# facebookresearch/wmar

Hardware: AMD Instinct MI355X
Metric: watermarked images/sec at 256x256 (16x16 tok), batch 64; detector p-value delta vs ref (higher is better)
Workload: dtype f32; 1 GPU; Taming cin_transformer (48L x 1536d x 24h, V=16384) + VQGAN f16/16384, 256x256, batch 64 per GPU, greenlist watermark delta=2 gamma=0.25 h=1 (linear/stratifiedrand), T=1 top-k 250 top-p 0.92; sample -> decode -> re-encode -> detect; random-init weights; batch_per_gpu=64, decode_loop=hipGraph replay, backend=nccl

## Files before the change

### wmar_amd/csrc/gpt.hip

```cpp
#include <cstdint>
#include <map>
#include <string>
#include <vector>

#include "decoder_host.h"
#include "decode_small.h"


using namespace wmar;

struct LayerW {
    float4 *wqkv, *wproj, *wfc1, *wfc2;
    float4* wfc1x16 = nullptr;
    float2* wfc1x8 = nullptr;
    float4* wqkvx_bx = nullptr;
    float4* wproj_bx = nullptr;
    float *bqkv, *bproj, *bfc1, *bfc2, *cqkv, *cfc1;
};

struct SmallW {
    float *wqkv = nullptr, *wproj = nullptr, *wfc1 = nullptr, *wfc2 = nullptr, *ln1w = nullptr, *ln2w = nullptr;
};

struct wmar_gpt {
// ... 15 lines not shown
    double* stats_q = nullptr;
    float *kcache = nullptr, *vcache = nullptr;
    float *logits = nullptr, *scratch = nullptr;
    long long* past = nullptr;
    int *pos_dev = nullptr, *step_dev = nullptr;
    hipEvent_t ev0 = nullptr;
    static constexpr int N_PHASE = 3;
    GraphSlots<N_PHASE> gr;
    GraphSlots<N_PHASE + 1> grh;
    unsigned long long hook_key[12] = {0};
    int att_nw = 2;
    unsigned long long graph_key[12] = {0};
    int att_t1 = 1 << 30, att_t2 = 1 << 30;
    bool att_user = false;
    int att_phase(int kv, int64_t B) const {
        if (!att_user && B * H < 512) return kv <= 128 ? 1 : 2;
        return kv <= att_t1 ? 0 : (kv <= att_t2 ? 1 : 2);
    }
    static int phase_waves(int ph) { return ph == 0 ? 1 : (ph == 1 ? 2 : 4); }
    int timing = 0;
    bool no_bx_qkv = false, no_bx_proj = false;
    unsigned* xsync = nullptr;
    bool xcd_ok = false;
    bool xcd_ok_created = false;
    bool no_xr = false;
    int inject_fail = 0;
    int fallbacks = 0;
    unsigned long long* dbg_sums = nullptr; int dbg_slot = 0;
    unsigned long long* stamps = nullptr;
    unsigned long long* stamp_slot(int l, int role) const {
        return stamps ? stamps + ((long long)(l * 5 + role) * WMAR_STAMP_UNITS) * 8 : nullptr;
    }
    bool no_bx = false;
    int force_s[3] = {0, 0, 0};
    double step_ms = 0.0;
    struct Span { int cls; hipEvent_t a, b; };
    std::vector<Span> spans;
    std::vector<hipEvent_t> ev_pool;
    size_t ev_used = 0;
    bool span_on = false;
    double cls_us[WMAR_T_NCLASS] = {0};
    int64_t cls_calls[WMAR_T_NCLASS] = {0};
    hipEvent_t next_event() {
        if (ev_used == ev_pool.size()) {
            hipEvent_t e = nullptr;
            (void)hipEventCreate(&e);
            ev_pool.push_back(e);
        }
        return ev_pool[ev_used++];
    }
    void span_begin(int cls, hipStream_t st) {
        if (!span_on) return;
        Span s{cls, next_event(), next_event()};
        (void)hipEventRecord(s.a, st);
        spans.push_back(s);
    }
    void span_end(hipStream_t st) {
        if (!span_on) return;
        (void)hipEventRecord(spans.back().b, st);
    }
    void span_collect() {
        for (int i = 0; i < WMAR_T_NCLASS; ++i) { cls_us[i] = 0; cls_calls[i] = 0; }
        for (auto& s : spans) {
            float ms = 0.f;
            if (hipEventElapsedTime(&ms, s.a, s.b) == hipSuccess) { cls_us[s.cls] += ms * 1000.0; cls_calls[s.cls] += 1; }
        }
// ... 53 lines not shown
        r.slabs = g->slabs; r.slab_stride = act;
        xcur = g->x;
        S_qkv = g->force_s[0] > 0 ? (g->force_s[0] > QKV_SLABS_MAX ? QKV_SLABS_MAX : g->force_s[0]) : 1;
        S_proj = g->force_s[1] > 0 ? g->force_s[1] : split_for(D / 32, KBD);
        S_fc2 = g->force_s[2] > 0 ? g->force_s[2] : ((MT % 2 == 0 && KBF >= 128) ? 4 : split_for(D / 32, KBF));
        if (g->force_s[2] <= 0 && MT == 2 && KBF >= 256) {
            const int NTd = D / 32;
            const int Slo = 256 / NTd;
            if (Slo >= 2 && Slo < MAX_SLABS && NTd * Slo <= 256) { S_fc2 = Slo; fc2_hi = 256 - NTd * Slo; if (fc2_hi >= NTd) fc2_hi = 0; }
        }
        const int NTq = 3 * D / 32;
        if (g->force_s[0] <= 0 && NTq % 4 == 0 && MT <= 2 && S_fc2 + (fc2_hi > 0 ? 1 : 0) <= MAX_SLABS) {
            const int G = NTq / 4;
            int S = 256 / G;
            if (S > QKV_SLABS_MAX) S = QKV_SLABS_MAX;
            if (S > KBD / QX_CK) S = KBD / QX_CK;
            if (S >= 1) S_qx = S;
        }
        proj_bx = MT == 2 && g->yq && g->layers[0].wproj_bx && !g->no_bx && !g->no_bx_proj && g->force_s[1] <= 0;
        if (proj_bx) S_proj = D / BX_KSLICE;
        proj_xr = xr_shape() && g->xcd_ok;
        nch_ln2 = proj_xr ? 16 : nch;
    }
    void dbg(const void* p, long long bytes) {
#ifdef WMAR_DEV_KNOBS
        if (!g->dbg_sums || g->dbg_slot >= 4096) return;
        hipLaunchKernelGGL(k_dbg_sum, dim3(512), dim3(256), 0, st, (const uint32_t*)p, bytes / 4, g->dbg_sums + g->dbg_slot++);
#else
        (void)p; (void)bytes;
#endif
    }
    bool xr_shape() const { return proj_bx && !g->no_xr && S_proj == 4 && (D / 32) % 8 == 0 && (D / 32 / 8) * S_proj <= 32 && (D / 32 / 8) % 2 == 0; }
    bool qkv_bx() const { return S_qx > 0 && MT == 2 && g->layers[0].wqkvx_bx && !g->no_bx && !g->no_bx_qkv; }
    bool fc1_x() const { return MT == 2 && g->layers[0].wfc1x16 && nch_ln2 <= 16; }
    int qx_nkeep() const { const int G = 3 * D / 128; return G >= 4 && S_qx * 4 <= STAT_CHUNKS_MAX ? 4 : 1; }
    bool head_ntw2() const { const int NT = g->V / 32; return MT == 2 && NT % 2 == 0 && NT / 2 <= 512; }
    int head_per() const { const int MG = (MT % 2 == 0) ? MT / 2 : MT; return 256 / MG > 0 ? 256 / MG : 1; }
    int split_for(int NT, int KB) const { return pick_split(MT % 2 == 0 ? NT * (MT / 2) : NT * MT, KB, 4); }
    GemmArgs base() const {
        GemmArgs a{};
        a.MT = MT; a.B = (int)B; a.stats = g->stats; a.n_chunks = nch; a.K = D;
        return a;
    }
    SgArgs sg_base() const {
        SgArgs a{};
        a.pos_dev = g->pos_dev; a.D = D; a.H = g->H; a.Tmax = g->Tmax;
        return a;
    }
    int embed() {
        if (small) {
            SeArgs e{g->tok_emb, g->pos_emb, g->xs, io.tok, io.tok_stride, io.tok_use_pos, g->pos_dev, D};
            g->span_begin(WMAR_T_EMBED, st);
            hipLaunchKernelGGL(k_sembed, dim3((unsigned)((D / 4 + 255) / 256), (unsigned)B), dim3(256), 0, st, e);
            g->span_end(st);
            return launch_status("k_sembed");
        }
        r.x = xcur;
        g->span_begin(WMAR_T_EMBED, st);
        hipLaunchKernelGGL((k_resid_stats<true, 0>), dim3(nch * MT), dim3(256), 0, st, r);
        g->span_end(st);
        return launch_status("k_resid_stats<embed>");
    }
    int resid(const float* bias, int S, int n_hi = 0) {
        r.x = xcur;
        r.S = S + (n_hi > 0 ? 1 : 0); r.bias = bias; r.n_hi = n_hi;
        g->span_begin(WMAR_T_RESID, st);
// ... 239 lines not shown
        const long long actb = act * 16, Mpad = MT * 32;
        const long long lstride = (long long)g->Bmax * g->H * g->Tmax * g->hd;
        switch (s) {
            case WMAR_GPT_STAGE_EMBED: dbg(xcur, actb); dbg(g->stats, nch * Mpad * 16); break;
            case WMAR_GPT_STAGE_QKV:
                if (S_qx > 0) { dbg(xcur, actb); dbg(g->stats_q, S_qx * Mpad * 16); dbg(g->qkv_slabs, S_qx * 3 * actb); }
                else { dbg(xcur, actb); dbg(g->stats, nch * Mpad * 16); dbg(g->qkv_slabs, 3 * actb); }
                break;
            case WMAR_GPT_STAGE_ATTN:
                if (proj_bx) dbg(g->yq, (long long)D / 16 * 2 * 3 * 64 * 16); else dbg(g->y, actb);
                dbg(g->kcache + l * lstride, lstride * 4); dbg(g->vcache + l * lstride, lstride * 4);
                break;
            case WMAR_GPT_STAGE_PROJ:
                dbg(g->slabs, S_proj * actb);
                if (proj_xr) { dbg(xcur, actb); dbg(g->stats, nch_ln2 * Mpad * 16); }
                break;
            case WMAR_GPT_STAGE_RESID_ATTN: dbg(xcur, actb); dbg(g->stats, nch_ln2 * Mpad * 16); break;
            case WMAR_GPT_STAGE_FC1: dbg(g->hbuf, 4 * actb); break;
            case WMAR_GPT_STAGE_FC2: dbg(g->slabs, S_fc2 * actb); break;
            case WMAR_GPT_STAGE_RESID_OUT: dbg(xcur, actb); dbg(g->stats, nch * Mpad * 16); break;
            default: break;
        }
    }
    int run_stages(int first, int last, int l) {
        for (int s = first; s <= last; ++s) {
            if (!has_stage(s, l)) continue;
            if (int rc = run_stage(s, l)) return rc;
            dbg_stage(s, l);
        }
        return WMAR_OK;
    }
};

int enqueue_step(wmar_gpt* g, int64_t B, const StepIO& io, hipStream_t st) {
    StepPlan p(g, B, io, st);
    int rc;
#ifdef WMAR_DEV_KNOBS
    if (g->dbg_sums) { g->dbg_slot = 0; if (hipMemsetAsync(g->dbg_sums, 0, 4096 * 8, st) != hipSuccess) return WMAR_EHIP; }
#endif
    if ((rc = p.run_stages(WMAR_GPT_STAGE_EMBED, WMAR_GPT_STAGE_EMBED, 0))) return rc;
    for (int l = 0; l < g->L; ++l)
        if ((rc = p.run_stages(WMAR_GPT_STAGE_RESID_IN, WMAR_GPT_STAGE_FC2, l))) return rc;
    return p.run_stages(WMAR_GPT_STAGE_RESID_OUT, WMAR_GPT_STAGE_HEAD, g->L - 1);
}

void note_replayed(wmar_gpt* g, int64_t B, const StepIO& io) {
    StepPlan pl(g, B, io, nullptr);
    if (!pl.small && pl.proj_xr) g->xr_enqueued = true;
}

}

extern "C" {

int wmar_gpt_create(const wmar_gpt_config* cfg, const char* const* names, const void* const* tensors_dev,
                    int32_t n_tensors, void* stream, wmar_gpt** out) {
    WMAR_REQUIRE(cfg && names && tensors_dev && out, "gpt_create: null argument");
    WMAR_REQUIRE(cfg->n_embd % cfg->n_head == 0, "n_embd %% n_head != 0");
    const int D = cfg->n_embd, H = cfg->n_head, hd = D / H, V = cfg->vocab_size, L = cfg->n_layer;
    WMAR_REQUIRE(D % 32 == 0 && V % 32 == 0 && D <= 8192, "n_embd (<= 8192) and vocab_size must be multiples of 32 (got %d, %d)", D, V);
    WMAR_REQUIRE(hd == 32 || hd == 64 || hd == 128, "head_dim %d unsupported (32, 64, 128)", hd);
    WMAR_REQUIRE(cfg->max_batch >= 1 && cfg->max_batch <= 128, "max_batch must be in 1..128");
    WMAR_REQUIRE(cfg->block_size >= 1 && L >= 1, "bad block_size / n_layer");
    TensorMap tm(names, tensors_dev, n_tensors);
    hipStream_t st = (hipStream_t)stream;
    auto* g = new wmar_gpt();
    g->cfg = *cfg; g->D = D; g->H = H; g->hd = hd; g->V = V; g->L = L; g->Tmax = cfg->block_size; g->Bmax = cfg->max_batch;
    g->MTmax = mt_for(cfg->max_batch);
#ifdef WMAR_DEV_KNOBS
    {
        const char* names_s[3] = {"WMAR_S_QKV", "WMAR_S_PROJ", "WMAR_S_FC2"};
        for (int i = 0; i < 3; ++i) {
            const char* e = getenv(names_s[i]);
            if (e) g->force_s[i] = atoi(e) > MAX_SLABS ? MAX_SLABS : atoi(e);
        }
    }
#endif
    g->no_bx = getenv("WMAR_NO_BX") != nullptr;
#ifdef WMAR_STAMPS
    if (getenv("WMAR_STAMPS")) {
        const size_t n = (size_t)L * 5 * WMAR_STAMP_UNITS * 8;
        if (hipMalloc(&g->stamps, n * 8) != hipSuccess || hipMemset(g->stamps, 0, n * 8) != hipSuccess) g->stamps = nullptr;
    }
#endif
#ifdef WMAR_DEV_KNOBS
    if (getenv("WMAR_DBG_SUMS")) { if (hipMalloc(&g->dbg_sums, 4096 * 8) != hipSuccess) g->dbg_sums = nullptr; }
    g->no_bx_qkv = getenv("WMAR_NO_BX_QKV") != nullptr; g->no_bx_proj = getenv("WMAR_NO_BX_PROJ") != nullptr;
#endif
    int& rc = tm.rc;
    const float* te = tm.need("tok_emb.weight");
    const float* pe = tm.need("pos_emb");
    const float* hw = tm.need("head.weight");
    const float *lfw = tm.need("ln_f.weight"), *lfb = tm.need("ln_f.bias");
    if (rc == WMAR_OK) {
        WMAR_TRY(copy_vec(g, &g->tok_emb, te, (size_t)V * D, st));
        WMAR_TRY(copy_vec(g, &g->pos_emb, pe, (size_t)cfg->block_size * D, st));
        WMAR_TRY(g->mem.alloc(&g->whead, (size_t)V * D / 4));
        WMAR_TRY(pack(hw, g->whead, V, D, 0, st, lfw));
        WMAR_TRY(g->mem.alloc(&g->bhead, (size_t)V));
        WMAR_TRY(fold_bias(hw, nullptr, lfb, g->bhead, V, D, st));
        WMAR_TRY(g->mem.alloc(&g->chead, (size_t)V));
        WMAR_TRY(fold_bias(hw, nullptr, lfw, g->chead, V, D, st));
    }
    g->layers.resize(L);
    for (int l = 0; l < L && rc == WMAR_OK; ++l) {
        std::string p = "blocks." + std::to_string(l) + ".";
        LayerW& w = g->layers[l];
        const float *qw = tm.need(p + "attn.query.weight"), *kw = tm.need(p + "attn.key.weight"), *vw = tm.need(p + "attn.value.weight");
        const float *qb = tm.need(p + "attn.query.bias"), *kb = tm.need(p + "attn.key.bias"), *vb = tm.need(p + "attn.value.bias");
        const float *pw = tm.need(p + "attn.proj.weight"), *pb = tm.need(p + "attn.proj.bias");
        const float *f1w = tm.need(p + "mlp.0.weight"), *f1b = tm.need(p + "mlp.0.bias");
// ... 190 lines not shown
            case WMAR_T_RESID: if (p.small) { set_error("profile_role: the small-batch path has no residual launch"); return WMAR_EINVAL; } return p.resid(g->layers[l].bproj, p.S_proj);
            case WMAR_T_FC1: return p.fc1(l);
            case WMAR_T_FC2: return p.fc2(l);
            case WMAR_T_HEAD: return p.head();
            default: set_error("profile_role: unknown role %d", role); return WMAR_EINVAL;
        }
    };
    const bool was = g->span_on;
    g->span_on = false;
    int rc = WMAR_OK;
    for (int i = 0; i < 3 && rc == WMAR_OK; ++i) rc = one(i);
    if (rc == WMAR_OK && hipEventRecord(g->ev0, st) != hipSuccess) rc = WMAR_EHIP;
    for (int i = 0; i < iters && rc == WMAR_OK; ++i) rc = one(i + 3);
    if (rc == WMAR_OK && hipEventRecord(g->gr.done, st) != hipSuccess) rc = WMAR_EHIP;
    g->span_on = was;
    if (rc) return rc;
    WMAR_HIP_CHECK(hipEventSynchronize(g->gr.done));
    float ms = 0.f;
    WMAR_HIP_CHECK(hipEventElapsedTime(&ms, g->ev0, g->gr.done));
    *avg_us = (double)ms * 1000.0 / iters;
    return WMAR_OK;
}

int wmar_gpt_plan_info(wmar_gpt* g, int64_t B, char* buf, int64_t buf_len) {
    WMAR_REQUIRE(g && buf && buf_len > 0, "plan_info: null argument");
    WMAR_REQUIRE(B >= 1 && B <= g->Bmax, "plan_info: batch outside 1..%d", g->Bmax);
    StepIO io{g->past, (long long)g->Tmax + 1, 0, g->logits};
    StepPlan p(g, B, io, nullptr);
    if (p.small) {
        const int n = snprintf(buf, (size_t)buf_len,
                               "qkv=k_sgemv<QKV> (row-major weight stream, LN1 + bias + cache append inside, %d columns per workgroup);"
                               "attn=k_sattn (4 waves per (sequence, head));proj=k_sgemv<PROJ> (residual added in place);resid=none;"
                               "resid_launches_per_step=0;fc1=k_sgemv<FC1> (LN2 + bias + GELU inside);fc2=k_sgemv<FC2> (8 K segments, residual added in place);"
                               "head=k_sgemv<HEAD> (ln_f inside);barrier_fallbacks=%d;path=small-batch streaming (decode_small.h)",
                               sg_cols_wg<3, 3, SG_QKV>(), g->fallbacks);
        WMAR_REQUIRE(n > 0 && n < buf_len, "plan_info: buffer of %lld bytes too small", (long long)buf_len);
        return WMAR_OK;
    }
    char qkv[96], proj[160], fc1[96], fc2[96];
    const int S_in = p.S_fc2 + (p.fc2_hi > 0 ? 1 : 0);
    if (p.qkv_bx()) snprintf(qkv, sizeof qkv, "k_qkvx_bx<%d> (bf16 pipe, %d K slices)", S_in, p.S_qx);
    else if (p.S_qx > 0) snprintf(qkv, sizeof qkv, "k_qkvx<%d,%d> (fp32 MFMA, %d K slices)", p.MT, S_in, p.S_qx);
    else snprintf(qkv, sizeof qkv, "k_gemm<EPI_PACKED> (fp32 MFMA, %d K slices) after k_resid_stats", p.S_qkv);
    if (p.proj_xr) snprintf(proj, sizeof proj, "k_bx_xr<%d,4> (bf16 pipe, 4 K slices + XCD-local reduction: residual fold and LN2 statistics inside)", BX_PER);
    else if (p.proj_bx) snprintf(proj, sizeof proj, "k_bx<1,%d> (bf16 pipe, %d K slices)", BX_PER, p.S_proj);
    else snprintf(proj, sizeof proj, "k_gemm<EPI_PACKED> (fp32 MFMA, %d K slices)", p.S_proj);
    if (p.fc1_x()) snprintf(fc1, sizeof fc1, "k_fc1x (fp32 MFMA, 24-column tiles, whole K)");
    else snprintf(fc1, sizeof fc1, "k_gemm<EPI_GELU,LN> (fp32 MFMA, whole K)");
    snprintf(fc2, sizeof fc2, "k_gemm<EPI_PACKED> (fp32 MFMA, %d%s K slices)", p.S_fc2, p.fc2_hi > 0 ? "/+1" : "");
    char attn[96];
    const int w0 = wmar_gpt::phase_waves(g->att_phase(1, B)), w1 = wmar_gpt::phase_waves(g->att_phase(g->Tmax / 2, B)),
              w2 = wmar_gpt::phase_waves(g->att_phase(g->Tmax, B));
    if (w0 == w1 && w1 == w2) snprintf(attn, sizeof attn, "k_attn_decode<%d,%d>", g->hd, w1);
    else snprintf(attn, sizeof attn, "k_attn_decode<%d,%d> (%d / %d / %d waves at 1 / %d / %d cached rows)", g->hd, w1, w0, w1, w2, g->Tmax / 2, g->Tmax);
    const int n = snprintf(buf, (size_t)buf_len, "qkv=%s;attn=%s;proj=%s;resid=k_resid_stats;resid_launches_per_step=%d;fc1=%s;fc2=%s;head=k_gemm<EPI_LOGITS,LN> (fp32 MFMA);barrier_fallbacks=%d",
                           qkv, attn, proj, p.proj_xr ? 1 : g->L + 1, fc1, fc2, g->fallbacks);
    WMAR_REQUIRE(n > 0 && n < buf_len, "plan_info: buffer of %lld bytes too small", (long long)buf_len);
    return WMAR_OK;
}

static const char* const kGptStageNames[] = {"EMBED", "RESID_IN", "QKV", "ATTN", "PROJ", "RESID_ATTN", "FC1", "FC2", "RESID_OUT", "HEAD"};

int wmar_gpt_probe_run(wmar_gpt* g, const int64_t* tok_dev, int64_t B, int32_t pos, int32_t layer, int32_t first_stage,
                       int32_t last_stage, float* logits_dev, void* stream) {
    WMAR_REQUIRE(g, "gpt_probe_run: null engine");
    WMAR_REQUIRE(B >= 1 && B <= g->Bmax, "gpt_probe_run: batch %lld outside 1..%d", (long long)B, g->Bmax);
    WMAR_REQUIRE(pos >= 0 && pos < g->Tmax, "gpt_probe_run: position %d outside the block size %d", pos, g->Tmax);
    WMAR_REQUIRE(layer >= 0 && layer < g->L, "gpt_probe_run: layer %d outside 0..%d", layer, g->L - 1);
    WMAR_REQUIRE(first_stage >= WMAR_GPT_STAGE_EMBED && last_stage <= WMAR_GPT_STAGE_HEAD && first_stage <= last_stage,
                 "gpt_probe_run: stages %d..%d", first_stage, last_stage);
    WMAR_REQUIRE(last_stage < WMAR_GPT_STAGE_HEAD || logits_dev, "gpt_probe_run: the HEAD stage needs logits_dev");
    WMAR_REQUIRE(first_stage > WMAR_GPT_STAGE_EMBED || tok_dev, "gpt_probe_run: the EMBED stage needs tok_dev");
    hipStream_t st = (hipStream_t)stream;
    StepIO io{(const long long*)tok_dev, 1, 0, logits_dev};
    g->att_nw = wmar_gpt::phase_waves(g->att_phase(pos + 1, B));
    StepPlan p(g, B, io, st);
    WMAR_REQUIRE(p.has_stage(first_stage, layer) && p.has_stage(last_stage, layer), "gpt_probe_run: the plan for %lld rows has no stage %s in block %d",
                 (long long)B, kGptStageNames[p.has_stage(first_stage, layer) ? last_stage : first_stage], layer);
    hipLaunchKernelGGL(k_set_int, dim3(1), dim3(1), 0, st, g->pos_dev, (int)pos);
    int rc = launch_status("k_set_int");
    for (int s = first_stage; s <= last_stage && rc == WMAR_OK; ++s) {
        if (!p.has_stage(s, layer)) continue;
        p.xcur = p.xcur_at(s, layer);
        rc = p.run_stage(s, layer);
    }
    const hipError_t e = hipStreamSynchronize(st);
    if (rc == WMAR_OK && e != hipSuccess) { set_error("gpt_probe_run: %s", hipGetErrorString(e)); rc = WMAR_EHIP; }
    if (rc != WMAR_OK) return rc;
    const int f = gpt_sync_failed(g, st);
    if (f < 0) return f;
    if (f > 0) {
        set_error("gpt_probe_run: the XCD-local barrier of the fused projection launch gave up or found a block on a foreign XCD: the stages "
                  "just run are invalid (the engine continues on the two-launch path)");
        return WMAR_EHIP;
    }
    return WMAR_OK;
}

int64_t wmar_gpt_probe_copy(wmar_gpt* g, const char* name, int32_t layer, void* ptr_dev, int64_t bytes, int32_t to_engine,
                            void* stream) {
    if (!g || !name) { set_error("gpt_probe_copy: null argument"); return WMAR_EINVAL; }
    if (layer < 0 || layer >= g->L) { set_error("gpt_probe_copy: layer %d outside 0..%d", layer, g->L - 1); return WMAR_EINVAL; }
    const std::string n = name;
    const size_t Mpad = (size_t)g->MTmax * 32, D = g->D, V = g->V;
    const size_t lkv = (size_t)g->Bmax * g->H * g->Tmax * g->hd;
    const size_t fx_units = (size_t)(4 * D / 24) * (D / 16) * 64;
    const LayerW& w = g->layers[layer];
    void* p = nullptr;
    size_t sz = 0;
    if (n == "x") { p = g->x; sz = Mpad * D * 4; }
    else if (n == "x2") { p = g->x2; sz = Mpad * D * 4; }
    else if (n == "y") { p = g->y; sz = Mpad * D * 4; }
    else if (n == "yq") { p = g->yq; sz = D / 16 * 2 * 3 * 64 * 16; }
    else if (n == "hbuf") { p = g->hbuf; sz = Mpad * 4 * D * 4; }
    else if (n == "slabs") { p = g->slabs; sz = (size_t)MAX_SLABS * Mpad * D * 4; }
    else if (n == "qkv_slabs") { p = g->qkv_slabs; sz = (size_t)MAX_SLABS * Mpad * 3 * D * 4; }
    else if (n == "stats") { p = g->stats; sz = (size_t)STAT_CHUNKS_MAX * Mpad * 2 * 8; }
    else if (n == "stats_q") { p = g->stats_q; sz = (size_t)QKV_SLABS_MAX * 4 * Mpad * 2 * 8; }
    else if (n == "kcache") { p = g->kcache + (size_t)layer * lkv; sz = lkv * 4; }
    else if (n == "vcache") { p = g->vcache + (size_t)layer * lkv; sz = lkv * 4; }
    else if (n == "xs") { p = g->xs; sz = (size_t)SG_MAX_ROWS * D * 4; }
    else if (n == "ys") { p = g->ys; sz = (size_t)SG_MAX_ROWS * D * 4; }
    else if (n == "qs") { p = g->qs; sz = (size_t)SG_MAX_ROWS * D * 4; }
    else if (n == "hs") { p = g->hs; sz = (size_t)SG_MAX_ROWS * 4 * D * 4; }
    else if (n == "wqkv") { p = w.wqkv; sz = 3 * D * D * 4; }
    else if (n == "wqkvx_bx") { p = w.wqkvx_bx; sz = 3 * D * D * 4; }
    else if (n == "wproj") { p = w.wproj; sz = D * D * 4; }
    else if (n == "wproj_bx") { p = w.wproj_bx; sz = D * D * 4; }
    else if (n == "wfc1") { p = w.wfc1; sz = 4 * D * D * 4; }
    else if (n == "wfc1x16") { p = w.wfc1x16; sz = fx_units * 16; }
    else if (n == "wfc1x8") { p = w.wfc1x8; sz = fx_units * 8; }
    else if (n == "wfc2") { p = w.wfc2; sz = 4 * D * D * 4; }
    else if (n == "bqkv") { p = w.bqkv; sz = 3 * D * 4; }
    else if (n == "cqkv") { p = w.cqkv; sz = 3 * D * 4; }
    else if (n == "bproj") { p = w.bproj; sz = D * 4; }
    else if (n == "bfc1") { p = w.bfc1; sz = 4 * D * 4; }
    else if (n == "cfc1") { p = w.cfc1; sz = 4 * D * 4; }
    else if (n == "bfc2") { p = w.bfc2; sz = D * 4; }
    else if (n == "whead") { p = g->whead; sz = V * D * 4; }
    else if (n == "bhead") { p = g->bhead; sz = V * 4; }
    else if (n == "chead") { p = g->chead; sz = V * 4; }
    else { set_error("gpt_probe_copy: unknown buffer '%s'", name); return WMAR_EINVAL; }
    if (!p) { set_error("gpt_probe_copy: this engine has no buffer '%s' (its shape is not eligible for the kernel that uses it)", name); return WMAR_EINVAL; }
    if (!ptr_dev) return (int64_t)sz;
    if (bytes != (int64_t)sz) { set_error("gpt_probe_copy: '%s' holds %zu bytes, caller passed %lld", name, sz, (long long)bytes); return WMAR_EINVAL; }
    hipStream_t st = (hipStream_t)stream;
    hipError_t e = to_engine ? hipMemcpyAsync(p, ptr_dev, sz, hipMemcpyDeviceToDevice, st)
                             : hipMemcpyAsync(ptr_dev, p, sz, hipMemcpyDeviceToDevice, st);
    if (e == hipSuccess) e = hipStreamSynchronize(st);
    if (e != hipSuccess) { set_error("gpt_probe_copy: %s", hipGetErrorString(e)); return WMAR_EHIP; }
// ... 92 lines not shown
}

int wmar_gpt_set_timing(wmar_gpt* g, int32_t enabled) { if (!g) return WMAR_EINVAL; g->timing = enabled; return WMAR_OK; }
int wmar_gpt_get_timing(wmar_gpt* g, double* total_us, int64_t* calls, double* step_ms) {
    if (!g) return WMAR_EINVAL;
    for (int i = 0; i < WMAR_T_NCLASS; ++i) {
        if (total_us) total_us[i] = g->cls_us[i];
        if (calls) calls[i] = g->cls_calls[i];
    }
    if (step_ms) *step_ms = g->step_ms;
    return WMAR_OK;
}

#ifndef WMAR_GRAPH_STEPS_DEFAULT
#define WMAR_GRAPH_STEPS_DEFAULT 4
#endif
static int gpt_generate_once(wmar_gpt* g, const wmar_wm_ctx* wm, const wmar_sample_params* sp, const int64_t* cond_dev,
                             int64_t B, int32_t steps, const float* q_dev, int64_t* tokens_out_dev,
                             float* logits_trace_dev, void* stream) {
    WMAR_REQUIRE(g && sp && cond_dev && q_dev && tokens_out_dev, "generate: null argument");
    WMAR_REQUIRE(B >= 1 && B <= g->Bmax, "generate: batch %lld outside 1..%d", (long long)B, g->Bmax);
    WMAR_REQUIRE(steps >= 1 && steps <= g->Tmax, "generate: steps %d outside 1..block_size %d", steps, g->Tmax);
    WMAR_REQUIRE(!(sp->top_p >= 0) || sp->top_p <= 1.0, "`top_p` has to be a float > 0 and < 1, but is %f", sp->top_p);
    if (wm) {
        WMAR_REQUIRE(wm->table_dev && wm->vocab_size == g->V, "generate: watermark vocab mismatch");
        WMAR_REQUIRE(wm->context_size >= 0 && wm->context_size <= WMAR_MAX_CONTEXT, "context size unsupported");
        WMAR_REQUIRE(wm->seed_strategy != WMAR_SEED_SPATIAL || wm->context_size == 1 || wm->context_size == 3,
                     "Spatial seeding only implemented for context size in [1,3]");
    }
    hipStream_t st = (hipStream_t)stream;
    const long long pstride = g->Tmax + 1;
    if (int rc = gpt_inject(g, st)) return rc;
    WMAR_HIP_CHECK(hipMemcpy2DAsync(g->past, pstride * 8, cond_dev, 8, 8, (size_t)B, hipMemcpyDeviceToDevice, st));
    WMAR_HIP_CHECK(hipMemsetAsync(g->pos_dev, 0, 8, st));

    SampArgs a{};
    a.wm = make_wm(wm);
    a.logits = g->logits; a.V = g->V; a.past = g->past; a.past_stride = pstride;
    a.t_dev = g->step_dev;
    a.temperature = sp->temperature; a.top_k = sp->top_k; a.use_top_p = sp->top_p >= 0;
    a.top_p_thr = (float)(1.0 - sp->top_p);
    a.q = q_dev; a.q_step_stride = (long long)B * g->V; a.step_dev = g->step_dev;
    a.scratch = a.V > 65536 ? g->scratch : nullptr;
    a.tok_out = (long long*)tokens_out_dev; a.tok_out_stride = steps;
    a.past_append = g->past; a.trace = logits_trace_dev; a.B = B;
    int* len_dev = g->pos_dev + 2;
    hipLaunchKernelGGL(k_set_int, dim3(1), dim3(1), 0, st, len_dev, 1);
    a.t_dev = len_dev;

    StepIO io{g->past, pstride, 1, g->logits};
    auto one_step = [&](hipStream_t s, int phase) -> int {
        g->att_nw = wmar_gpt::phase_waves(phase);
        int rc = enqueue_step(g, B, io, s);
        if (rc) return rc;
        g->span_begin(WMAR_T_SAMPLE, s);
        rc = launch_sample_fused(a, s);
        g->span_end(s);
        if (rc) return rc;
        hipLaunchKernelGGL(k_advance3, dim3(1), dim3(1), 0, s, g->pos_dev);
        return launch_status("k_advance3");
    };

    if (g->timing) WMAR_HIP_CHECK(hipEventRecord(g->ev0, st));
    if (sp->use_graph) {
        unsigned long long key[12] = {(unsigned long long)B, (unsigned long long)steps, (unsigned long long)(uintptr_t)q_dev,
                                      (unsigned long long)(uintptr_t)tokens_out_dev, (unsigned long long)(uintptr_t)logits_trace_dev,
                                      wm ? (unsigned long long)(uintptr_t)wm->table_dev : 0ull,
                                      wm ? (unsigned long long)wm->n_rows : 0ull,
                                      wm ? ((unsigned long long)wm->seed_strategy << 40) | ((unsigned long long)wm->context_size << 20) | (unsigned long long)wm->spatial_dim : 0ull,
                                      0ull, 0ull, (unsigned long long)sp->top_k, 0ull};
        float fd = wm ? wm->delta : 0.f, ft = sp->temperature;
        memcpy(&key[8], &fd, 4); memcpy(&key[9], &ft, 4); memcpy(&key[11], &sp->top_p, 8);
        bool need[wmar_gpt::N_PHASE] = {false, false, false};
        for (int n = 0; n < steps; ++n) need[g->att_phase(n + 1, B)] = true;
        int gs = 1;
        {
            const int want = WMAR_GRAPH_STEPS_DEFAULT;
            const int n_need = (int)need[0] + (int)need[1] + (int)need[2];
            if (n_need == 1 && want > 1 && steps % want == 0) gs = want;
        }
        key[1] |= (unsigned long long)gs << 32;
        if (memcmp(key, g->graph_key, sizeof(key)) != 0) g->gr.drop();
        bool have = true;
        for (int ph = 0; ph < wmar_gpt::N_PHASE; ++ph) have = have && (!need[ph] || g->gr.exec[ph]);
        if (!have) {
            g->gr.drop();
            for (int ph = 0; ph < wmar_gpt::N_PHASE; ++ph) {
                if (!need[ph]) continue;
                const int rc = g->gr.capture(ph, [&](hipStream_t s) {
                    int r = WMAR_OK;
                    for (int k = 0; k < gs && r == WMAR_OK; ++k) r = one_step(s, ph);
                    return r;
                });
                if (rc) return rc;
            }
            memcpy(g->graph_key, key, sizeof(key));
        }
        for (int n = 0; n < steps; n += gs)
            if (int rc = g->gr.replay(g->att_phase(n + 1, B), st)) return rc;
        if (int rc = g->gr.replayed(st)) return rc;
        note_replayed(g, B, io);
        if (g->timing) WMAR_HIP_CHECK(hipEventSynchronize(g->gr.done));
    } else {
        g->span_on = g->timing != 0;
        int rc = WMAR_OK;
        for (int n = 0; n < steps && rc == WMAR_OK; ++n) rc = one_step(st, g->att_phase(n + 1, B));
        g->span_on = false;
        if (rc) return rc;
        if (g->timing) {
            WMAR_HIP_CHECK(hipEventRecord(g->gr.done, st));
            WMAR_HIP_CHECK(hipStreamSynchronize(st));
            g->span_collect();
        }
    }
    if (g->timing) {
        float ms = 0;
        WMAR_HIP_CHECK(hipEventElapsedTime(&ms, g->ev0, g->gr.done));
        g->step_ms = ms / steps;
    }
    return WMAR_OK;
}

int wmar_gpt_generate(wmar_gpt* g, const wmar_wm_ctx* wm, const wmar_sample_params* sp, const int64_t* cond_dev,
                      int64_t B, int32_t steps, const float* q_dev, int64_t* tokens_out_dev,
                      float* logits_trace_dev, void* stream) {
    WMAR_REQUIRE(g, "generate: null argument");
    return run_with_fallback("generate: the in-launch barrier flag is up on the two-launch path",
                             [&] { return gpt_generate_once(g, wm, sp, cond_dev, B, steps, q_dev, tokens_out_dev, logits_trace_dev, stream); },
                             [&] { return gpt_sync_failed(g, (hipStream_t)stream); });
}

static int gpt_generate_hooked_once(wmar_gpt* g, const wmar_sample_params* sp, const int64_t* cond_dev, int64_t B, int32_t steps,
                                    const float* q_dev, int64_t* tokens_out_dev, const HookIO& hk, void* stream) {
    WMAR_REQUIRE(g && sp && cond_dev && q_dev && tokens_out_dev && hk.logits && hk.past && hk.hook, "generate_hooked: null argument");
    WMAR_REQUIRE(B >= 1 && B <= g->Bmax, "generate_hooked: batch %lld outside 1..%d", (long long)B, g->Bmax);
    WMAR_REQUIRE(steps >= 1 && steps <= g->Tmax, "generate_hooked: steps %d outside 1..block_size %d", steps, g->Tmax);
    WMAR_REQUIRE(hk.past_stride >= (long long)steps + 1, "generate_hooked: past_stride %lld below steps + 1 = %d", hk.past_stride, steps + 1);
    WMAR_REQUIRE(!(sp->top_p >= 0) || sp->top_p <= 1.0, "`top_p` has to be a float > 0 and < 1, but is %f", sp->top_p);
// ... 76 lines not shown
```

### wmar_amd/csrc/sampler.h

```cpp
#pragma once
#include "common.h"

namespace wmar {

struct WmDev {
    const uint32_t* table;
    long long n_rows;
    long long row_words;
    int seed_mode, h, S;
    float delta;
    int enabled;
};

inline WmDev make_wm(const wmar_wm_ctx* wm) {
    WmDev d{};
    if (wm) {
        d.table = wm->table_dev;
        d.n_rows = wm->n_rows;
        d.row_words = (wm->vocab_size + 31) / 32;
        d.seed_mode = wm->seed_strategy;
        d.h = wm->context_size;
        d.S = wm->spatial_dim;
        d.delta = wm->delta;
        d.enabled = 1;
    }
    return d;
}

struct SampArgs {
    WmDev wm;
    const float* logits;
    long long V;
    const long long* past;
    long long past_stride;
    long long t_host;
    const int* t_dev;
    float temperature;
    int top_k;
    int use_top_p;
    float top_p_thr;
    const float* q;
    long long q_step_stride;
    const int* step_dev;
    float* scratch;
    long long* tok_out;
    long long tok_out_stride;
    long long* past_append;
    float* trace;
    long long B;
    const float* logits_uncond;
    const float* cfg_scale;
    const float* logits_img;
    float g_text, g_image;
    const uint32_t* allow;
    const int* gather;
    long long Vsrc;
};

int launch_sample_fused(const SampArgs& a, hipStream_t st);

struct CfgMixArgs {
    const float* cond;
    const float* img;
    const float* uncond;
    float* out;
    long long V, B;
    const float* scale;
    const int* step_dev;
    float g_text, g_image;
};

int launch_cfg_mix(const CfgMixArgs& a, hipStream_t st);

struct HookIO {
    float* logits;
    long long* past;
    long long past_stride;
    wmar_logits_hook hook;
    void* user;
};

inline int call_hook(const HookIO& h, int step, long long t) {
    const int r = h.hook(h.user, (int32_t)step, (int64_t)t);
    if (r != 0) { set_error("the logits hook returned %d at step %d: generation stopped", r, step); return WMAR_ECALLBACK; }
    return WMAR_OK;
}

struct GumbelArgs {
    const float* logits;
// ... 33 lines not shown
```

### wmar_amd/csrc/watermark.hip

```cpp
#include "sampler.h"
#include "../../include/wmar_math.h"

namespace wmar {

__device__ __forceinline__ const uint32_t* wm_row(const WmDev& wm, const long long* past, long long t) {
    if (!wm.enabled) return nullptr;
    long long r = ctx_row(past, t, wm.seed_mode, wm.h, wm.S);
    if (r < 0 || r >= wm.n_rows) return nullptr;
    return wm.table + r * wm.row_words;
}

__global__ __launch_bounds__(256) void k_wm_bias(WmDev wm, float* logits, long long V, const long long* past,
                                                 long long t, long long past_stride) {
    const long long b = blockIdx.y;
    const uint32_t* row = wm_row(wm, past + b * past_stride, t);
    if (!row) return;
    float* lg = logits + b * V;
    const float d = wm.delta;
    for (long long w = blockIdx.x * blockDim.x + threadIdx.x; w * 32 < V; w += (long long)gridDim.x * blockDim.x) {
        uint32_t bits = row[w];
        if (!bits) continue;
        long long v0 = w * 32;
        for (int j = 0; j < 32 && v0 + j < V; ++j)
            if ((bits >> j) & 1u) lg[v0 + j] = lg[v0 + j] + d;
// ... 33 lines not shown
            if (three) {
                const float4 m = i4[i];
                r.x = cfg_mix3(c.x, m.x, u.x, a.g_text, a.g_image); r.y = cfg_mix3(c.y, m.y, u.y, a.g_text, a.g_image);
                r.z = cfg_mix3(c.z, m.z, u.z, a.g_text, a.g_image); r.w = cfg_mix3(c.w, m.w, u.w, a.g_text, a.g_image);
            } else {
                r.x = cfg_mix2(c.x, u.x, scale); r.y = cfg_mix2(c.y, u.y, scale);
                r.z = cfg_mix2(c.z, u.z, scale); r.w = cfg_mix2(c.w, u.w, scale);
            }
            o4[i] = r;
        }
    } else {
        for (long long v = (long long)blockIdx.x * blockDim.x + threadIdx.x; v < a.V; v += stride) {
            const float c = a.cond[off + v], u = a.uncond[off + v];
            a.out[off + v] = three ? cfg_mix3(c, a.img[off + v], u, a.g_text, a.g_image) : cfg_mix2(c, u, scale);
        }
    }
}

int launch_cfg_mix(const CfgMixArgs& a, hipStream_t st) {
    const auto al = [](const void* p) { return (reinterpret_cast<uintptr_t>(p) & 15u) == 0; };
    const bool vec = a.V % 4 == 0 && al(a.cond) && al(a.uncond) && al(a.out) && (!a.img || al(a.img));
    const long long per_row = vec ? a.V / 4 : a.V;
    long long gx = (per_row + 255) / 256;
    if (gx > 64) gx = 64;
    if (gx < 1) gx = 1;
    const dim3 grid((unsigned)gx, (unsigned)a.B);
    if (vec) hipLaunchKernelGGL(k_cfg_mix<true>, grid, dim3(256), 0, st, a);
    else hipLaunchKernelGGL(k_cfg_mix<false>, grid, dim3(256), 0, st, a);
    return launch_status("k_cfg_mix");
}

constexpr int SAMP_THREADS = 1024;
constexpr int SAMP_WAVES = SAMP_THREADS / 64;

__device__ __forceinline__ unsigned long long wave_sum_u64(unsigned long long v) {
    for (int o = 32; o > 0; o >>= 1) v += __shfl_xor(v, o);
    return v;
}

__device__ __forceinline__ unsigned long long block_sum_u64(unsigned long long v, unsigned long long* red) {
    v = wave_sum_u64(v);
    const int w = threadIdx.x >> 6, l = threadIdx.x & 63;
    if (l == 0) red[w] = v;
    __syncthreads();
    unsigned long long s = 0;
    for (int i = 0; i < SAMP_WAVES; ++i) s += red[i];
    return s;
}

__device__ __forceinline__ uint32_t block_max_u32(uint32_t v, unsigned long long* red) {
    for (int o = 32; o > 0; o >>= 1) v = max(v, (uint32_t)__shfl_xor((int)v, o));
    const int w = threadIdx.x >> 6, l = threadIdx.x & 63;
    if (l == 0) red[w] = v;
    __syncthreads();
    uint32_t s = 0;
    for (int i = 0; i < SAMP_WAVES; ++i) s = max(s, (uint32_t)red[i]);
    return s;
}

template <bool ASC_MASS>
__device__ __forceinline__ int scan_hist(const unsigned long long* hist, unsigned long long need_or_base, float thr,
                                         unsigned long long* other) {
    const int l = threadIdx.x & 63;
    unsigned long long h0, h1, h2, h3;
    if (ASC_MASS) {
        h0 = hist[4 * l], h1 = hist[4 * l + 1], h2 = hist[4 * l + 2], h3 = hist[4 * l + 3];
// ... 375 lines not shown
#pragma unroll
            for (int j = 0; j < CH; ++j) {
                const int i = c0 + j;
                const long long v = tid + (long long)i * SAMP_THREADS;
                if (v < V) {
                    const float xv = xr[i];
                    const uint32_t k = wmar_f32_key(xv);
                    const bool kept = k >= thr_key && (k > bkey || (k == bkey && v >= bidx));
                    const float e = kept ? wmar_expf(xv - m) : 0.0f;
                    const float r = (e / Sf2) / qv[j];
                    if (r > best) { best = r; besti = (int)v; }
                }
            }
        }
    } else {
        for (long long v = tid; v < V; v += SAMP_THREADS) {
            const float xv = x[v];
            const uint32_t k = wmar_f32_key(xv);
            const bool kept = k >= thr_key && (k > bkey || (k == bkey && v >= bidx));
            const float e = kept ? wmar_expf(xv - m) : 0.0f;
            const float r = (e / Sf2) / q[WMAR_SRC(v)];
            if (r > best) { best = r; besti = (int)v; }
        }
    }
    }
#undef WMAR_FOR_ROW
    for (int o = 32; o > 0; o >>= 1) {
        float ob = __shfl_xor(best, o);
        int oi = __shfl_xor(besti, o);
        if (ob > best || (ob == best && oi < besti)) { best = ob; besti = oi; }
    }
    if ((tid & 63) == 0) { red_f[tid >> 6] = best; red_i[tid >> 6] = besti; }
    __syncthreads();
    if (tid == 0) {
        for (int i = 1; i < SAMP_WAVES; ++i)
            if (red_f[i] > best || (red_f[i] == best && red_i[i] < besti)) { best = red_f[i]; besti = red_i[i]; }
        const long long tokv = WMAR_SRC(besti);
        a.tok_out[b * a.tok_out_stride + step] = tokv;
        if (a.past_append) a.past_append[b * a.past_stride + t] = tokv;
    }
#undef WMAR_SRC
}

struct DetArgs {
    WmDev wm;
    double gamma;
    const long long* codes;
    long long L;
    int* n_scored;
    int* n_green;
    double* pval;
    signed char* mask;
    long long mask_stride;
};

__device__ __forceinline__ long long det_num_ngrams(int seed_mode, int h, long long L, long long S) {
    if (seed_mode != WMAR_SEED_SPATIAL) return L - h;
    if (h == 1) return L - 1;
    return (S - 1) * (S - 1);
}

__device__ __forceinline__ void det_ngram_pos(int seed_mode, int h, long long S, long long i, long long* pos) {
    if (seed_mode != WMAR_SEED_SPATIAL) {
        for (int j = 0; j <= h; ++j) pos[j] = i + j;
    } else if (h == 1) {
        long long cell = i + 1;
        long long r = cell / S, c = cell % S;
        pos[0] = (c == 0) ? (r - 1) * S : cell - 1;
        pos[1] = cell;
    } else {
        long long r = i / (S - 1), c = i % (S - 1);
        pos[0] = r * S + c; pos[1] = r * S + c + 1; pos[2] = (r + 1) * S + c; pos[3] = (r + 1) * S + c + 1;
// ... 241 lines not shown
```

Before: 59.42 images/s.

## Fuse next-step embedding, stats and counter advance into sampling kernel

The sampling kernel now writes the next step's input rows (token plus position embedding in the tiled layout) and their per-chunk LayerNorm statistics itself. It also advances the position counters through an atomic last-block election, so the separate k_advance3 and embed launches drop out of each decode step. The first step's embedding is issued once before graph replay. This removes two small launches per step from the graph, at the cost of extra work and complexity in the sampler tail and reliance on atomic counter ordering.

```diff
diff --git a/wmar_amd/csrc/gpt.hip b/wmar_amd/csrc/gpt.hip
--- a/wmar_amd/csrc/gpt.hip
+++ b/wmar_amd/csrc/gpt.hip
@@ -71,6 +71,7 @@
         return stamps ? stamps + ((long long)(l * 5 + role) * WMAR_STAMP_UNITS) * 8 : nullptr;
     }
     bool no_bx = false;
+    bool no_sample_embed = false;
     int force_s[3] = {0, 0, 0};
     double step_ms = 0.0;
     struct Span { int cls; hipEvent_t a, b; };
@@ -190,6 +191,7 @@
     }
     bool xr_shape() const { return proj_bx && !g->no_xr && S_proj == 4 && (D / 32) % 8 == 0 && (D / 32 / 8) * S_proj <= 32 && (D / 32 / 8) % 2 == 0; }
     bool qkv_bx() const { return S_qx > 0 && MT == 2 && g->layers[0].wqkvx_bx && !g->no_bx && !g->no_bx_qkv; }
+    bool tail_fused() const { return !small && !g->no_sample_embed; }
     bool fc1_x() const { return MT == 2 && g->layers[0].wfc1x16 && nch_ln2 <= 16; }
     int qx_nkeep() const { const int G = 3 * D / 128; return G >= 4 && S_qx * 4 <= STAT_CHUNKS_MAX ? 4 : 1; }
     bool head_ntw2() const { const int NT = g->V / 32; return MT == 2 && NT % 2 == 0 && NT / 2 <= 512; }
@@ -495,13 +497,13 @@
     }
 };
 
-int enqueue_step(wmar_gpt* g, int64_t B, const StepIO& io, hipStream_t st) {
+int enqueue_step(wmar_gpt* g, int64_t B, const StepIO& io, hipStream_t st, bool have_embed = false) {
     StepPlan p(g, B, io, st);
     int rc;
 #ifdef WMAR_DEV_KNOBS
-    if (g->dbg_sums) { g->dbg_slot = 0; if (hipMemsetAsync(g->dbg_sums, 0, 4096 * 8, st) != hipSuccess) return WMAR_EHIP; }
+    if (g->dbg_sums) { g->dbg_slot = have_embed ? 2 : 0; if (hipMemsetAsync(g->dbg_sums, 0, 4096 * 8, st) != hipSuccess) return WMAR_EHIP; }
 #endif
-    if ((rc = p.run_stages(WMAR_GPT_STAGE_EMBED, WMAR_GPT_STAGE_EMBED, 0))) return rc;
+    if (!have_embed && (rc = p.run_stages(WMAR_GPT_STAGE_EMBED, WMAR_GPT_STAGE_EMBED, 0))) return rc;
     for (int l = 0; l < g->L; ++l)
         if ((rc = p.run_stages(WMAR_GPT_STAGE_RESID_IN, WMAR_GPT_STAGE_FC2, l))) return rc;
     return p.run_stages(WMAR_GPT_STAGE_RESID_OUT, WMAR_GPT_STAGE_HEAD, g->L - 1);
@@ -540,6 +542,7 @@
     }
 #endif
     g->no_bx = getenv("WMAR_NO_BX") != nullptr;
+    g->no_sample_embed = getenv("WMAR_NO_SAMPLE_EMBED") != nullptr;
 #ifdef WMAR_STAMPS
     if (getenv("WMAR_STAMPS")) {
         const size_t n = (size_t)L * 5 * WMAR_STAMP_UNITS * 8;
@@ -796,7 +799,8 @@
                                "qkv=k_sgemv<QKV> (row-major weight stream, LN1 + bias + cache append inside, %d columns per workgroup);"
                                "attn=k_sattn (4 waves per (sequence, head));proj=k_sgemv<PROJ> (residual added in place);resid=none;"
                                "resid_launches_per_step=0;fc1=k_sgemv<FC1> (LN2 + bias + GELU inside);fc2=k_sgemv<FC2> (8 K segments, residual added in place);"
-                               "head=k_sgemv<HEAD> (ln_f inside);barrier_fallbacks=%d;path=small-batch streaming (decode_small.h)",
+                               "head=k_sgemv<HEAD> (ln_f inside);barrier_fallbacks=%d;path=small-batch streaming (decode_small.h);"
+                               "tail=k_sample_fused, k_advance3, k_sembed (three launches)",
                                sg_cols_wg<3, 3, SG_QKV>(), g->fallbacks);
         WMAR_REQUIRE(n > 0 && n < buf_len, "plan_info: buffer of %lld bytes too small", (long long)buf_len);
         return WMAR_OK;
@@ -817,8 +821,10 @@
               w2 = wmar_gpt::phase_waves(g->att_phase(g->Tmax, B));
     if (w0 == w1 && w1 == w2) snprintf(attn, sizeof attn, "k_attn_decode<%d,%d>", g->hd, w1);
     else snprintf(attn, sizeof attn, "k_attn_decode<%d,%d> (%d / %d / %d waves at 1 / %d / %d cached rows)", g->hd, w1, w0, w1, w2, g->Tmax / 2, g->Tmax);
-    const int n = snprintf(buf, (size_t)buf_len, "qkv=%s;attn=%s;proj=%s;resid=k_resid_stats;resid_launches_per_step=%d;fc1=%s;fc2=%s;head=k_gemm<EPI_LOGITS,LN> (fp32 MFMA);barrier_fallbacks=%d",
-                           qkv, attn, proj, p.proj_xr ? 1 : g->L + 1, fc1, fc2, g->fallbacks);
+    const int n = snprintf(buf, (size_t)buf_len, "qkv=%s;attn=%s;proj=%s;resid=k_resid_stats;resid_launches_per_step=%d;fc1=%s;fc2=%s;head=k_gemm<EPI_LOGITS,LN> (fp32 MFMA);barrier_fallbacks=%d;tail=%s",
+                           qkv, attn, proj, p.proj_xr ? 1 : g->L + 1, fc1, fc2, g->fallbacks,
+                           p.tail_fused() ? "k_sample_fused (one launch: next step's input rows, statistics and the counters inside, generate only)"
+                                          : "k_sample_fused, k_advance3, k_resid_stats<embed> (three launches)");
     WMAR_REQUIRE(n > 0 && n < buf_len, "plan_info: buffer of %lld bytes too small", (long long)buf_len);
     return WMAR_OK;
 }
@@ -880,6 +886,7 @@
     else if (n == "slabs") { p = g->slabs; sz = (size_t)MAX_SLABS * Mpad * D * 4; }
     else if (n == "qkv_slabs") { p = g->qkv_slabs; sz = (size_t)MAX_SLABS * Mpad * 3 * D * 4; }
     else if (n == "stats") { p = g->stats; sz = (size_t)STAT_CHUNKS_MAX * Mpad * 2 * 8; }
+    else if (n == "ctr") { p = g->pos_dev; sz = 16; }
     else if (n == "stats_q") { p = g->stats_q; sz = (size_t)QKV_SLABS_MAX * 4 * Mpad * 2 * 8; }
     else if (n == "kcache") { p = g->kcache + (size_t)layer * lkv; sz = lkv * 4; }
     else if (n == "vcache") { p = g->vcache + (size_t)layer * lkv; sz = lkv * 4; }
@@ -1038,7 +1045,7 @@
     const long long pstride = g->Tmax + 1;
     if (int rc = gpt_inject(g, st)) return rc;
     WMAR_HIP_CHECK(hipMemcpy2DAsync(g->past, pstride * 8, cond_dev, 8, 8, (size_t)B, hipMemcpyDeviceToDevice, st));
-    WMAR_HIP_CHECK(hipMemsetAsync(g->pos_dev, 0, 8, st));
+    WMAR_HIP_CHECK(hipMemsetAsync(g->pos_dev, 0, 16, st));
 
     SampArgs a{};
     a.wm = make_wm(wm);
@@ -1055,14 +1062,21 @@
     a.t_dev = len_dev;
 
     StepIO io{g->past, pstride, 1, g->logits};
+    const StepPlan pl(g, B, io, nullptr);
+    const bool fused = pl.tail_fused();
+    if (fused) {
+        a.emb_tok = g->tok_emb; a.emb_pos = g->pos_emb; a.emb_x = g->x; a.emb_stats = g->stats;
+        a.emb_K = g->D; a.emb_MT = pl.MT; a.emb_nch = pl.nch; a.emb_Tmax = g->Tmax; a.ctr = g->pos_dev;
+    }
+    auto first_embed = [&](hipStream_t s) -> int { return fused ? StepPlan(g, B, io, s).embed() : WMAR_OK; };
     auto one_step = [&](hipStream_t s, int phase) -> int {
         g->att_nw = wmar_gpt::phase_waves(phase);
-        int rc = enqueue_step(g, B, io, s);
+        int rc = enqueue_step(g, B, io, s, fused);
         if (rc) return rc;
         g->span_begin(WMAR_T_SAMPLE, s);
         rc = launch_sample_fused(a, s);
         g->span_end(s);
-        if (rc) return rc;
+        if (rc || fused) return rc;
         hipLaunchKernelGGL(k_advance3, dim3(1), dim3(1), 0, s, g->pos_dev);
         return launch_status("k_advance3");
     };
@@ -1085,7 +1099,7 @@
             const int n_need = (int)need[0] + (int)need[1] + (int)need[2];
             if (n_need == 1 && want > 1 && steps % want == 0) gs = want;
         }
-        key[1] |= (unsigned long long)gs << 32;
+        key[1] |= (unsigned long long)gs << 32 | (unsigned long long)(fused ? 1 : 0) << 48;
         if (memcmp(key, g->graph_key, sizeof(key)) != 0) g->gr.drop();
         bool have = true;
         for (int ph = 0; ph < wmar_gpt::N_PHASE; ++ph) have = have && (!need[ph] || g->gr.exec[ph]);
@@ -1102,6 +1116,7 @@
             }
             memcpy(g->graph_key, key, sizeof(key));
         }
+        if (int rc = first_embed(st)) return rc;
         for (int n = 0; n < steps; n += gs)
             if (int rc = g->gr.replay(g->att_phase(n + 1, B), st)) return rc;
         if (int rc = g->gr.replayed(st)) return rc;
@@ -1109,7 +1124,7 @@
         if (g->timing) WMAR_HIP_CHECK(hipEventSynchronize(g->gr.done));
     } else {
         g->span_on = g->timing != 0;
-        int rc = WMAR_OK;
+        int rc = first_embed(st);
         for (int n = 0; n < steps && rc == WMAR_OK; ++n) rc = one_step(st, g->att_phase(n + 1, B));
         g->span_on = false;
         if (rc) return rc;
diff --git a/wmar_amd/csrc/sampler.h b/wmar_amd/csrc/sampler.h
--- a/wmar_amd/csrc/sampler.h
+++ b/wmar_amd/csrc/sampler.h
@@ -55,6 +55,12 @@
     const uint32_t* allow;
     const int* gather;
     long long Vsrc;
+    const float* emb_tok;
+    const float* emb_pos;
+    float4* emb_x;
+    double* emb_stats;
+    int emb_K, emb_MT, emb_nch, emb_Tmax;
+    int* ctr;
 };
 
 int launch_sample_fused(const SampArgs& a, hipStream_t st);
diff --git a/wmar_amd/csrc/watermark.hip b/wmar_amd/csrc/watermark.hip
--- a/wmar_amd/csrc/watermark.hip
+++ b/wmar_amd/csrc/watermark.hip
@@ -89,6 +89,7 @@
 
 constexpr int SAMP_THREADS = 1024;
 constexpr int SAMP_WAVES = SAMP_THREADS / 64;
+constexpr int SAMP_EMB_CHUNKS = 64;
 
 __device__ __forceinline__ unsigned long long wave_sum_u64(unsigned long long v) {
     for (int o = 32; o > 0; o >>= 1) v += __shfl_xor(v, o);
@@ -530,12 +531,69 @@
     }
     if ((tid & 63) == 0) { red_f[tid >> 6] = best; red_i[tid >> 6] = besti; }
     __syncthreads();
+    if (a.ctr && tid == SAMP_THREADS - 1) {
+        if (__hip_atomic_fetch_add(a.ctr + 3, 1, __ATOMIC_RELAXED, __HIP_MEMORY_SCOPE_AGENT) == (int)a.B - 1) {
+            __hip_atomic_fetch_add(a.ctr + 0, 1, __ATOMIC_RELAXED, __HIP_MEMORY_SCOPE_AGENT);
+            __hip_atomic_fetch_add(a.ctr + 1, 1, __ATOMIC_RELAXED, __HIP_MEMORY_SCOPE_AGENT);
+            __hip_atomic_fetch_add(a.ctr + 2, 1, __ATOMIC_RELAXED, __HIP_MEMORY_SCOPE_AGENT);
+            __hip_atomic_store(a.ctr + 3, 0, __ATOMIC_RELAXED, __HIP_MEMORY_SCOPE_AGENT);
+        }
+    }
     if (tid == 0) {
         for (int i = 1; i < SAMP_WAVES; ++i)
             if (red_f[i] > best || (red_f[i] == best && red_i[i] < besti)) { best = red_f[i]; besti = red_i[i]; }
         const long long tokv = WMAR_SRC(besti);
         a.tok_out[b * a.tok_out_stride + step] = tokv;
         if (a.past_append) a.past_append[b * a.past_stride + t] = tokv;
+    }
+    static_assert(SAMP_WAVES == 16 && 64 + SAMP_EMB_CHUNKS * 8 <= SAMP_THREADS, "k_sample_fused: hand-over thread layout");
+    if (a.emb_x && t < (long long)a.emb_Tmax) {
+        const int KB = a.emb_K / 8, nch = a.emb_nch, MT = a.emb_MT, j = tid - 64;
+        if (j >= 0 && (j & ~63) < nch * 8) {
+            float wb = red_f[tid & 15];
+            int wi = red_i[tid & 15];
+            for (int o = 8; o > 0; o >>= 1) {
+                const float ob = __shfl_xor(wb, o);
+                const int oi = __shfl_xor(wi, o);
+                if (ob > wb || (ob == wb && oi < wi)) { wb = ob; wi = oi; }
+            }
+            if (j < nch * 8) {
+                const long long tokv = WMAR_SRC(wi);
+                const int c = j >> 3, w = (j >> 1) & 3, half = j & 1;
+                const int kb0 = (int)((long long)c * KB / nch), kb1 = (int)((long long)(c + 1) * KB / nch);
+                const int mt = (int)(b >> 5), lane = (int)(b & 31) + 32 * half;
+                const float* erow = a.emb_tok + tokv * a.emb_K;
+                const float* prow = a.emb_pos + t * a.emb_K;
+                float4 v[4], bb[4];
+                int kbs[4];
+#pragma unroll
+                for (int i = 0; i < 4; ++i) {
+                    const int kb = kb0 + w + 4 * i;
+                    kbs[i] = kb < kb1 ? kb : -1;
+                    const int k = (kb < kb1 ? kb : kb0) * 8 + 4 * half;
+                    v[i] = *(const float4*)(erow + k);
+                    bb[i] = *(const float4*)(prow + k);
+                }
+                double s = 0.0, ss = 0.0;
+#pragma unroll
+                for (int i = 0; i < 4; ++i) {
+                    if (kbs[i] < 0) continue;
+                    const float4 r = make_float4(v[i].x + bb[i].x, v[i].y + bb[i].y, v[i].z + bb[i].z, v[i].w + bb[i].w);
+                    a.emb_x[((long long)kbs[i] * MT + mt) * 64 + lane] = r;
+                    s += (double)r.x + (double)r.y + (double)r.z + (double)r.w;
+                    ss += sq4_f64(r);
+                }
+                const double ps = s + __shfl_xor(s, 1), pss = ss + __shfl_xor(ss, 1);
+                const int base = tid & 56;
+                double ts = 0, tss = 0;
+#pragma unroll
+                for (int i = 0; i < 4; ++i) { ts += __shfl(ps, base + 2 * i); tss += __shfl(pss, base + 2 * i); }
+                if ((j & 7) == 0) {
+                    double* o = a.emb_stats + ((long long)c * (MT * 32) + b) * 2;
+                    o[0] = ts; o[1] = tss;
+                }
+            }
+        }
     }
 #undef WMAR_SRC
 }
```

After: 59.84 images/s (median of 3 runs). About the same (+0.7%).
